# zhong-yy/volpick

Hardware: AMD Instinct MI355X
Metric: waveform-windows/sec (higher is better)
Workload: dtype f32 (exact 3xbf16 split products, fp32 accumulate)

## Files before the change

### include/volpick_hip.h

```cpp
#ifndef VOLPICK_HIP_H
#define VOLPICK_HIP_H

#include <stddef.h>
#include <stdint.h>

#ifdef __cplusplus
extern "C" {
#endif

typedef struct vp_handle vp_handle;

typedef enum {
  VP_OK = 0,
  VP_ERR_INVALID = -1,
  VP_ERR_HIP = -2,
  VP_ERR_NOMEM = -3,
  VP_ERR_UNSUPPORTED = -4
} vp_status;

enum { VP_MODEL_PHASENET = 0, VP_MODEL_EQTRANSFORMER = 1 };
enum { VP_NORM_PEAK = 0, VP_NORM_STD = 1 };
enum { VP_STACK_AVG = 0, VP_STACK_MAX = 1 };
enum { VP_MEM_HOST = 0, VP_MEM_DEVICE = 1 };

// ... 85 lines not shown
int vp_step_issued_work(const vp_handle* h, int index, vp_issued_work* out);
int vp_step_issued_work_for_range(const vp_handle* h, int index, int out_lo, int out_hi, vp_issued_work* out);
int vp_profile_steps(vp_handle* h, int B, int iters, float* step_ms, int cap);
int vp_profile_step_in_pipeline(vp_handle* h, int B, int iters, int index, float* ms);
int vp_profile_one_step(vp_handle* h, int B, int iters, int index, float* ms);

int vp_debug_plan_conv(int model_kind, const float* weights, size_t n_floats, const vp_config* cfg,
                       int conv_index, int* geom13, float* afrag, size_t afrag_cap, float* bias, size_t bias_cap,
                       const char** name, int* cols, int* l_out);

int vp_debug_tensor_count(const vp_handle* h);
int vp_debug_tensor_info(const vp_handle* h, int index, const char** name, int* channels, int* length);
int vp_debug_tensor_read(vp_handle* h, int index, int B, float* host_out);

int vp_debug_check_halos(vp_handle* h, int self_test, int64_t* n_bad, const char** first_bad_tensor);

int vp_debug_core_clock(vp_handle* h, int B, unsigned long long* out32);
int vp_debug_conv_clock(vp_handle* h, unsigned long long* out, int max_layers);
int vp_debug_tail_clock(vp_handle* h, int B, unsigned long long* out32);

enum { VP_SAMPLES_INT32 = 0, VP_SAMPLES_FLOAT32 = 1 };
typedef struct {
  int64_t offset;
  int64_t start_us;
  double sample_rate;
  int32_t reclen, data_offset, nsamples, encoding;
  int32_t big_endian;
  int32_t quality;
  char network[4], station[8], location[4], channel[4];
} vp_mseed_record;
// ... 111 lines not shown
```

### volpick_amd/_lib.py

```python
from __future__ import annotations

import ctypes as C
import os
from pathlib import Path

_HERE = Path(__file__).resolve().parent
LIB_PATH = Path(os.environ.get("VOLPICK_HIP_LIB", _HERE / "libvolpick_hip.so"))

VP_MODEL_PHASENET, VP_MODEL_EQTRANSFORMER = 0, 1
VP_TRAIN_FP32, VP_TRAIN_BF16 = 0, 1
VP_NORM_PEAK, VP_NORM_STD = 0, 1
VP_STACK_AVG, VP_STACK_MAX = 0, 1
VP_MEM_HOST, VP_MEM_DEVICE = 0, 1
VP_MAX_INFLIGHT = 4
VP_ABI_VERSION = 3


class VpConfig(C.Structure):
    _fields_ = [
        ("norm", C.c_int32),
        ("norm_amp_per_comp", C.c_int32),
        ("max_batch", C.c_int32),
        ("bn_eps", C.c_float),
        ("attention_eps", C.c_float),
# ... 216 lines not shown
    "vp_bank_destroy": (C.c_int, [_H]),
    "vp_bank_make_batch": (
        C.c_int, [_H, C.c_void_p, C.c_int, C.c_int, C.c_float, C.c_int, C.POINTER(C.c_int), C.c_void_p, C.c_void_p, C.c_void_p],
    ),
    "vp_train_step_bank": (
        C.c_int,
        [_H, _H, C.c_void_p, C.c_int, C.c_float, C.c_int, C.POINTER(C.c_int), C.c_float, C.c_int, C.POINTER(C.c_double)],
    ),
    "vp_bank_make_batch_aug": (
        C.c_int, [_H, C.c_void_p, C.c_int, C.c_int, C.c_float, C.c_int, C.POINTER(C.c_int), C.c_void_p, C.c_void_p, C.c_void_p],
    ),
    "vp_train_step_bank_aug": (
        C.c_int,
        [_H, _H, C.c_void_p, C.c_int, C.c_float, C.c_int, C.POINTER(C.c_int), C.c_float, C.c_int, C.POINTER(C.c_double)],
    ),
    "vp_last_error": (C.c_char_p, []),
    "vp_version": (C.c_char_p, []),
}


def load():
    global _lib
    if _lib is not None:
        return _lib
    if not LIB_PATH.exists():
        raise VolpickHipError(
            f"{LIB_PATH} not found: the HIP extension is required (no CPU fallback). "
            f"Build it with `make -C {_HERE / 'csrc'}` or `python -c 'import __graft_entry__ as g; g.build()'`."
        )
    try:
# ... 25 lines not shown
```

### volpick_amd/csrc/api.hip

```cpp
#include <algorithm>
#include <cmath>
#include <mutex>
#include <numeric>

#include "net.h"
#include "prepost.h"

namespace vp {
const char* last_error();
}

struct vp_handle {
  int device = 0;
  hipStream_t stream = nullptr;
  vp::Net net;
  hipEvent_t ev[5] = {};
  float total_ms = 0.f;
  bool timing = false;
  float stage_ms[4] = {0.f, 0.f, 0.f, 0.f};
  vp::PreArgs last_pre{};
  int last_pre_windows = 0;
  int last_out_lo = 0, last_out_hi = 0;
  float* d_in = nullptr;
  size_t d_in_cap = 0;
// ... 1076 lines not shown
int vp_debug_tensor_read(vp_handle* h, int index, int B, float* host_out) {
  VP_REQUIRE(h && host_out && index >= 0 && index < (int)h->net.tensors.size(), "bad argument");
  const vp::Tensor& t = h->net.tensors[index];
  if (h->net.tensor_sets[index] == 0) {
    vp::set_error("tensor %s is not materialised by this plan", t.name.c_str());
    return VP_ERR_UNSUPPORTED;
  }
  VP_REQUIRE(B > 0 && B <= h->net.max_batch * h->net.tensor_sets[index], "bad B");
  VP_HIP(hipSetDevice(h->device));
  VP_HIP(hipStreamSynchronize(h->stream));
  VP_HIP(hipMemcpy2D(host_out, (size_t)t.L * sizeof(float), t.p + vp::HALO, (size_t)t.ls * sizeof(float),
                     (size_t)t.L * sizeof(float), (size_t)B * t.C, hipMemcpyDeviceToHost));
  return VP_OK;
}

int vp_debug_check_halos(vp_handle* h, int self_test, int64_t* n_bad, const char** first_bad_tensor) {
  VP_REQUIRE(h && n_bad, "null argument");
  VP_HIP(hipSetDevice(h->device));
  vp::Net& net = h->net;
  const size_t nt = net.tensors.size();
  VP_REQUIRE(self_test >= 0 && self_test <= (int)nt, "self_test names tensor %d of %zu", self_test - 1, nt);
  float* planted = nullptr;
  if (self_test > 0) {
    const vp::Tensor& t = net.tensors[self_test - 1];
    const size_t rows = (size_t)t.C * net.max_batch * net.tensor_sets[self_test - 1];
    VP_REQUIRE(rows > 0, "tensor %s is not materialised by this plan", t.name.c_str());
    planted = t.p + (rows - 1) * t.ls + vp::HALO + t.L;
    const float one = 1.f;
    VP_HIP(hipMemcpyAsync(planted, &one, sizeof(float), hipMemcpyHostToDevice, h->stream));
  }
// ... 85 lines not shown
```

### volpick_amd/csrc/eqt.hip

```cpp
#include "eqt_kernels.h"
#include "net.h"

namespace vp {

namespace {

using EQ_e0 = ConvCfg<3, 0, 8, 2, 12, 2, -5, 0, 1, 4, 8, 1, EPI_POOL2, 1>;
using EQ_e1 = ConvCfg<8, 0, 16, 1, 9, 1, -4, 0, 1, 4, 8, 1, EPI_POOL2, 1>;
using EQ_e2 = ConvCfg<16, 0, 16, 1, 7, 1, -3, 0, 1, 4, 6, 1, EPI_POOL2>;
using EQ_e3 = ConvCfg<16, 0, 32, 1, 7, 1, -3, 0, 2, 2, 6, 1, EPI_POOL2>;
using EQ_e4 = ConvCfg<32, 0, 32, 1, 5, 1, -2, 0, 2, 2, 6, 1, EPI_POOL2, 0, 1>;
using EQ_e5 = ConvCfg<32, 0, 64, 1, 5, 1, -2, 0, 4, 1, 6, 1, EPI_POOL2, 0, 1>;
using EQ_e6 = ConvCfg<64, 0, 64, 1, 3, 1, -1, 0, 4, 1, 3, 1, EPI_POOL2_DUAL, 0, 1>;
using EQ_r1k3 = ConvCfg<64, 0, 64, 1, 3, 1, -1, 0, 4, 1, 3, 1, EPI_STORE>;
using EQ_r1k2 = ConvCfg<64, 0, 64, 1, 2, 1, 0, 0, 4, 1, 3, 1, EPI_STORE>;
using EQ_r2k3 = ConvCfg<64, 0, 64, 1, 3, 1, -1, 0, 4, 1, 3, 0, EPI_RES>;
using EQ_r2k2 = ConvCfg<64, 0, 64, 1, 2, 1, 0, 0, 4, 1, 3, 0, EPI_RES>;
using EQ_d0 = ConvCfg<16, 0, 64, 2, 3, 1, -1, 0, 4, 1, 3, 1, EPI_STORE>;
using EQ_d1 = ConvCfg<64, 0, 64, 2, 3, 1, -1, 0, 4, 1, 6, 1, EPI_STORE, 0, 1>;
using EQ_d2 = ConvCfg<64, 0, 32, 2, 3, 1, -1, 0, 2, 2, 6, 1, EPI_STORE, 0, 1>;
using EQ_d3 = ConvCfg<32, 0, 32, 2, 5, 1, -2, 0, 2, 2, 6, 1, EPI_STORE>;
using EQ_d4 = ConvCfg<32, 0, 16, 2, 5, 1, -2, 0, 2, 2, 6, 1, EPI_STORE, 0, 1>;
using EQ_d5 = ConvCfg<16, 0, 16, 2, 5, 1, -2, 0, 2, 2, 6, 1, EPI_STORE, 0, 1>;
using EQ_d6 = ConvCfg<16, 0, 8, 2, 7, 1, -3, 0, 1, 4, 6, 1, EPI_HEAD, 1>;
// ... 442 lines not shown
    for (int d = 0; d < 3; ++d) {
      const float* hw = pv.get(std::string(head[d]) + ".weight");
      L->e0.h.insert(L->e0.h.end(), hw, hw + 88);
      L->e1.h.push_back(pv.get(std::string(head[d]) + ".bias")[0]);
    }
    L->flops_per_window += 3 * 2.0 * 8 * 11 * T;
    net.steps.back().flops_per_window = L->flops_per_window;
    net.steps.back().name = "decoder.6+heads";
    L->name = "decoder.6";
  }

  net.flops_per_window = 0;
  for (auto& s : net.steps) net.flops_per_window += s.flops_per_window;
  if (net.cfg.plan_flags[1] & 2)
    net.debug_clock = net.add_blob(std::vector<float>(((size_t)net.max_batch * 64 + 64 * 8) * 2, 0.f));
  if (net.cfg.plan_flags[0] != 1) {
    int rc = plan_eqt_fuse_res(net);
    if (rc != VP_OK) return rc;
  }
  if (!(net.cfg.plan_flags[7] & 1) && !alt) {
    int rc = (net.cfg.plan_flags[7] & 64) ? plan_eqt_fuse_tail(net) : plan_eqt_fuse_tail_b3(net);
    if (rc != VP_OK) return rc;
  }
  if (!(net.cfg.plan_flags[7] & 4)) {
    int rc = plan_eqt_fuse_front(net, !(net.cfg.plan_flags[7] & 256));
    if (rc != VP_OK) return rc;
  }
  if (!(net.cfg.plan_flags[7] & 8)) {
    int rc = (net.cfg.plan_flags[7] & 128) ? plan_eqt_fuse_enc36(net) : plan_eqt_fuse_enc36_b3(net);
    if (rc != VP_OK) return rc;
// ... 10 lines not shown
```

### volpick_amd/csrc/eqt_front.hip

```cpp
#include <type_traits>

#include "conv_b3.h"
#include "conv_lds.h"
#include "eqt_kernels.h"
#include "net.h"
#include "prepost.h"

namespace vp {

namespace {

constexpr int FR_NTH = 512, FR_WAVES = 8;
constexpr int FW = 250, FR_TILES = 3;
constexpr int T_IN = 6000, L0P = 3000, L1P = 1500;
using F_e0 = LdsLayer<3, 0, 8, 2, 12, 2, -5, 0, 8, 1>;
using F_e1 = LdsLayer<8, 0, 16, 1, 9, 1, -4, 0, 8, 1>;
using F_e2 = LdsLayer<16, 0, 16, 1, 7, 1, -3, 0, 4, 1>;
constexpr int C0 = 1024, C1 = 1024, C2 = 512;
constexpr int SI = 2065, BII = 8, S0P = 1040, S1P = 528, BI = 4;
static_assert(SI % 32 == 17 && S0P % 32 == 16 && S1P % 32 == 16, "bank-conflict-free strides");
static_assert(SI >= BII + 2 * (C0 - 1) + 12 - 5 && S0P >= BI + C1 + 4 && S0P >= C0 && S1P >= BI + C2 + 3 && S1P >= 1 + C1 / 2,
              "image widths");
constexpr int OFFI = 0, OFF0P = 4 * SI + 4 - (4 * SI) % 4, OFF1P = OFF0P + 8 * S0P, FR_LDS_FLOATS = OFF1P + 16 * S1P;
static_assert(FR_LDS_FLOATS * 4 <= 160 * 1024 && OFF0P % 4 == 0 && OFF1P % 4 == 0, "LDS budget");
// ... 9 lines not shown

struct FrontArgs {
  const float* x;
  int ls_x;
  long ws_x;
  float* y;
  int ls_y;
  long ws_y;
  const float* af[3];
  const float* bs[3];
  const uint4* af3[2];
  int n_tiles;
  PreArgs pre;
  int has_pre;
  int B;
};
struct FrontDumpArgs : FrontArgs {
  float* dbg[2];
  int dbg_ls[2];
  long dbg_ws[2];
};

__device__ __forceinline__ void front_window_stats(const PreArgs& p, const float* src, const long cs, float* red, float* out) {
  constexpr int VT = 1024, NWV = 16, MAXE = 6;
  const int tid = threadIdx.x, lane = tid & 63, wave = tid >> 6, T = p.T;
  float* stat = red + 3 * NWV;
  if (p.norm == VP_NORM_PEAK) {
    float s[2][3], hi[3] = {-INFINITY, -INFINITY, -INFINITY}, lo[3] = {INFINITY, INFINITY, INFINITY};
#pragma unroll
    for (int h = 0; h < 2; ++h)
// ... 222 lines not shown
  float* lds = reinterpret_cast<float*>(fr_lds_raw);
  int off0 = OFF0P / 4, off1 = OFF1P / 4;
  asm volatile("" : "+v"(off0), "+v"(off1));
  float* XI = lds + OFFI;
  float* E0P = lds + 4 * off0;
  float* E1P = lds + 4 * off1;
  bf16_t* E0 = reinterpret_cast<bf16_t*>(reinterpret_cast<char*>(fr_lds_raw) + FB_OFF_E0);
  bf16_t* E1 = reinterpret_cast<bf16_t*>(reinterpret_cast<char*>(fr_lds_raw) + FB_OFF_E1);
  __shared__ float fr_red[3 * 16 + 8 + 3 * 16];
  __shared__ float fr_stat[8];
  const int tid = threadIdx.x, lane = tid & 63;
  const int wave_u = __builtin_amdgcn_readfirstlane(tid >> 6);
  constexpr bool has_pre = CUT;
  int seq = 0;
  auto tile_at = [&](const int q) {
    return has_pre ? ((int)blockIdx.x + (q / FR_TILES) * (int)gridDim.x) * FR_TILES + q % FR_TILES : (int)blockIdx.x + q * (int)gridDim.x;
  };
  int tile = tile_at(0);
  if (tile >= a.n_tiles) return;
  for (int i = tid; i < SI + 4; i += FR_NTH) XI[3 * SI + i] = 0.f;
  if constexpr (B3) {
    uint4* z = reinterpret_cast<uint4*>(reinterpret_cast<char*>(fr_lds_raw) + FB_OFF_E0);
    for (int i = tid; i < (FB_LDS_BYTES - FB_OFF_E0) / 16; i += FR_NTH) z[i] = make_uint4(0u, 0u, 0u, 0u);
  }

  float pre[PRE];
  auto raw_window = [&](const int win, long& cs) -> const float* {
    const PreArgs& p = a.pre;
    long start = p.dense ? 0 : (long)(p.first_window + win) * p.step;
    if (!p.dense && start > p.N - T_IN) start = p.N - T_IN;
    const float* src = p.src + (p.dense ? (long)win * 3 * T_IN : start);
// ... 193 lines not shown
  st.run = [=](Net& n, int B, hipStream_t s) -> int {
    FrontArgs a{};
    const Tensor &tx = n.tensors[x_in], &ty = n.tensors[y_out];
    a.x = tx.p;
    a.ls_x = tx.ls;
    a.ws_x = (long)tx.win_stride();
    a.y = ty.p;
    a.ls_y = ty.ls;
    a.ws_y = (long)ty.win_stride();
    for (int i = 0; i < 3; ++i) {
      a.af[i] = c[i]->afrag.d;
      a.bs[i] = c[i]->bias.d;
    }
    a.n_tiles = B * FR_TILES;
    a.B = B;
    if (n.pre) {
      a.pre = *n.pre;
      a.has_pre = 1;
    }
    const int grid = a.has_pre ? (B < 256 ? B : 256) : (a.n_tiles < 256 ? a.n_tiles : 256);
    if (b3) {
      for (int i = 0; i < 2; ++i) a.af3[i] = reinterpret_cast<const uint4*>(p3[i]->d);
      if (dumps) {
        if (a.has_pre) {
          set_error("fused encoder front: dumps with the in-kernel preprocessing");
          return VP_ERR_UNSUPPORTED;
        }
        FrontDumpArgs d{};
        static_cast<FrontArgs&>(d) = a;
        for (int i = 0; i < 2; ++i) {
// ... 34 lines not shown
```

### volpick_amd/csrc/phasenet_arena.h

```cpp
#pragma once
#include "conv_lds.h"
#include "conv_valu.h"
#include "net.h"

namespace vp {

constexpr int T0 = 3001, T1 = 751, T2 = 188, T3 = 47, T4 = 12;
constexpr int IB = 4;

constexpr int img_stride(int L) { return ((4 + L + 20 - 16 + 31) / 32) * 32 + 16; }
constexpr int S1_ = img_stride(T1), S2_ = img_stride(T2), S3_ = img_stride(T3), S4_ = img_stride(T4);
static_assert(S1_ == 784 && S2_ == 240 && S3_ == 80 && S4_ == 48, "image strides");

template <int C, int S, int L, int B = IB>
__device__ __forceinline__ void zero_halo(float* img, int tid, int nth) {
  constexpr int RW = S - L;
  for (int i = tid; i < C * RW; i += nth) {
    const int c = i / RW, k = i - c * RW;
    img[c * S + (k < B ? k : L + k)] = 0.f;
  }
}

template <int S, int B>
struct RangeStore {
// ... 166 lines not shown
  const uint4* af3_u3t;
  const uint4* af3_u3s;
  const float *bs_u3t, *bs_u3s;
  const float* x;
  int ls_x;
  long ws_x;
  float* skip0;
  int ls_s;
  long ws_s;
  float* y;
  const f32x2 *w_inc, *b_inc, *w_same, *b_same, *w_up, *b_up;
  const float *af_down, *bs_down, *af_t, *bs_t;
  const float *w_out, *b_out;
  PreArgs pre;
  int has_pre;
  float* dbg[WD_COUNT];
  int dbg_ls[WD_COUNT];
  long dbg_ws[WD_COUNT];
};

enum class PnForm {
  Default,
  Level0Valu,
  Fp32Core,
};

void pn_launch_down0(const Down0Args& a, int B, hipStream_t s);
void pn_launch_down0v(const Down0VArgs& a, int B, hipStream_t s);
void pn_launch_core(const CoreArgs& a, int B, hipStream_t s);
void pn_launch_up3(const Up3Args& a, int B, bool persistent, hipStream_t s);
// ... 7 lines not shown
```

### volpick_amd/csrc/phasenet_fused.hip

```cpp
#include "phasenet_arena.h"

namespace vp {

namespace {

int tensor_id(const Net& net, const std::string& name) {
  for (size_t i = 0; i < net.tensors.size(); ++i)
    if (net.tensors[i].name == name) return (int)i;
  return -1;
}

std::vector<float> pack_valu(const float* W, int cin, bool transposed, const std::vector<float>& scale) {
  std::vector<float> out((size_t)cin * 7 * 8);
  for (int ci = 0; ci < cin; ++ci)
    for (int k = 0; k < 7; ++k)
      for (int co = 0; co < 8; ++co)
        out[((size_t)ci * 7 + k) * 8 + co] = scale[co] * (transposed ? W[((size_t)ci * 8 + co) * 7 + k] : W[((size_t)co * cin + ci) * 7 + k]);
  return out;
}

std::vector<float> pack_u2same_half(const ConvLayer& L, int half) {
  const int taps = L.g.taps;
  std::vector<uint16_t> o((size_t)4 * 3 * 64 * 8);
  for (int st = 0; st < 4; ++st)
// ... 217 lines not shown
    a.b_inc = pairs(p.vb[0]);
    a.w_same = pairs(p.vw[1]);
    a.b_same = pairs(p.vb[1]);
    a.w_up = pairs(p.vw[4]);
    a.b_up = pairs(p.vb[4]);
    a.af_down = n.convs[2]->afrag.d;
    a.bs_down = n.convs[2]->bias.d;
    a.af_t = n.convs[16]->afrag.d;
    a.bs_t = n.convs[16]->bias.d;
    a.w_out = e0->d;
    a.b_out = e1->d;
    if (n.pre) {
      a.pre = *n.pre;
      a.has_pre = 1;
    }
    for (size_t i = 0; i < wd_ids.size(); ++i) bind(n.tensors[wd_ids[i]], &a.dbg[i], &a.dbg_ls[i], &a.dbg_ws[i]);
    pn_launch_window(form, !wd_ids.empty(), a, B, s);
    return 0;
  };
  return st;
}

}

int plan_phasenet_fused(Net& net, const ParamView& pv, int debug_flags) {
  PnPlan p{};
  p.debug_dumps = (debug_flags & 1) != 0;
  p.debug_clock = (debug_flags & 2) != 0;
  const bool win_dumps = (debug_flags & 4) != 0;
  const int f5 = net.cfg.plan_flags[5];
  if (win_dumps && (p.debug_dumps || f5 != 0 || net.cfg.plan_flags[6] != 0)) {
    set_error("PhaseNet plan_flags[1] & 4 dumps the default one-launch form only (plan_flags[1] & 1, plan_flags[5], plan_flags[6] unset)");
    return VP_ERR_UNSUPPORTED;
  }
  if (net.cfg.plan_flags[2] == 1 || f5 == 4 || f5 == 5 || f5 == 6 || f5 == 7 || f5 == 9) {
    set_error("PhaseNet plan_flags[2] = %d / plan_flags[5] = %d: this A/B form was removed in round 6 (kept: plan_flags[5] = 0, 1, 2, 3, 8)",
              net.cfg.plan_flags[2], f5);
    return VP_ERR_UNSUPPORTED;
  }
  if (net.cfg.plan_flags[3] == 2) {
    set_error("PhaseNet plan_flags[3] = 2 (persistent level-0 down kernel): removed in round 6");
    return VP_ERR_UNSUPPORTED;
  }
  p.valu = f5 != 1;
  p.persistent = net.cfg.plan_flags[3] != 1;
  const bool whole = p.valu && f5 != 2 && !p.debug_dumps;
  const PnForm form = f5 == 3 ? PnForm::Fp32Core : f5 == 8 ? PnForm::Level0Valu : PnForm::Default;
  if (p.valu) {
    const float eps = net.cfg.bn_eps;
    struct {
      const char *conv, *bn;
      int cin;
      bool transposed, bias;
    } spec[5] = {{"inc", "in_bn", 3, false, true},
                 {"down_branch.0.0", "down_branch.0.1", 8, false, false},
                 {"down_branch.0.2", "down_branch.0.3", 8, false, false},
// ... 60 lines not shown
```

### volpick_amd/csrc/phasenet_window.hip

```cpp
#include "conv_b3.h"
#include "phasenet_arena.h"

namespace vp {

namespace {

constexpr int W0_Q = W0_S / 4;
constexpr int W_LANES = (T0 + 3) / 4;
constexpr int W_WAVES = (W0_Q + 63) / 64;
constexpr int WD_H = 0, WD_X = 8 * W0_S;
static_assert(11 * W0_S <= CORE_LDS_FLOATS, "level-0 down images must fit the core arena");
static_assert(WD_X <= A_D0 && A_D0 + 8 * S1_ <= 11 * W0_S, "down0.down lands on the dead x rows");
constexpr int WU_U = A_SKIP2, WU_G0 = 0, WU_G1 = WU_U + 16 * S1_;
static_assert(WU_G0 + 4 * W0_S <= WU_U && WU_U + 16 * S1_ <= A_U2T && WU_G1 + 4 * W0_S <= CORE_LDS_FLOATS, "up-phase regions");
using W_down = LdsLayer<8, 0, 8, 2, 11, 8, -3, 0, 1, 1>;
using W_upT = LdsLayer<16, 0, 8, 4, 2, 1, -1, -2, 3, 1>;

__device__ __forceinline__ float* win_dump_row(const WindowArgs& a, const int i, const int win, const int c) {
  return a.dbg[i] + (long)win * a.dbg_ws[i] + HALO + (long)c * a.dbg_ls[i];
}
__device__ __forceinline__ float b3_join(const bf16_t* p, const int ps) {
  return from_bf16(p[0]) + (from_bf16(p[ps]) + from_bf16(p[2 * ps]));
}
template <int C, int S, int B>
// ... 47 lines not shown
constexpr int B3_U1_NC = 200, B3_U1_PS = B3_U1_NC * 40;
static_assert(A_U2T * 4 % 16 == 0 && A_U2T * 2 + 3 * B3_U1_PS <= CORE_LDS_FLOATS * 2 && B3_U1_NC >= 192 + 6, "up1.same piece image");
constexpr int B3_U0S_NC = 50, B3_U0S_PS = B3_U0S_NC * 72;
constexpr int B3_U0T_SHIFT = ((A_Q * 2 + 3 * B3_U0S_PS - A_R * 2 + 7) / 8) * 8;
constexpr int B3_U1S_NC = 194;
constexpr int B3_U2_NC = 768, B3_U2_OFF = (A_SKIP2 * 4 + 3 * B3Chunk<32, B3_U1S_NC>::PS * 2 + 15) / 16 * 4;
static_assert(B3_U0T_SHIFT >= 0 && A_R * 2 + B3_U0T_SHIFT + 3 * B3_U0T_PS <= B3_SK3_OFF && (A_R * 2 + B3_U0T_SHIFT) % 8 == 0,
              "up0.convT's image between up0.same's output pieces and the skip-3 image");
static_assert(B3_U2_OFF * 4 + 3 * B3Chunk<16, B3_U2_NC>::PS * 2 <= CORE_LDS_FLOATS * 4 && B3_U2_NC >= 47 * 16 + 8 + 3 &&
                  B3_U1S_NC >= 192 + 2,
              "up1.same's output pieces and up2.same's image behind them fit the arena");
constexpr int B3_D0_NC = 760, B3_D1_NC = 200;
static_assert(A_D0 * 4 + 3 * B3Chunk<8, B3_D0_NC>::PS * 2 <= CORE_LDS_FLOATS * 4 && B3_D0_NC >= 47 * 16 + 7 && B3_D1_NC >= 192 + 7,
              "down0.down / down1.down as piece images");
constexpr int D0T_TS = 512, D0T_RING = 1040, D0T_HPS = B3Chunk<8, D0T_RING>::PS;
constexpr int D0T_RED = CORE_LDS_FLOATS - 256;
static_assert(D0T_TILES * D0T_TS >= W0_S - 4 + 8 && D0T_RING >= 2 * D0T_TS + 11 + 4 && D0T_RING % 2 == 0 &&
                  WD_X * 4 + 3 * D0T_HPS * 2 <= D0T_RED * 4 && (9 * 16 + 8) <= 256,
              "level-0 tiles: the ring behind the eight fp32 rows, the scratch behind the ring, inside the arena");
constexpr int U3T_TS = 256, U3T_RING = 528, U3T_NCU = 768;
using U3T_QU = B3Chunk<16, U3T_NCU>;
constexpr int U3T_PLN = U3T_RING / 2, U3T_MIR = 4;
constexpr int U3T_PL = (U3T_PLN + U3T_MIR) * 8, U3T_CH = 2 * U3T_PL, U3T_PS = 2 * U3T_CH;
constexpr int U3T_RING_OFF = 3 * U3T_QU::PS;
static_assert(U3T_TILES * U3T_TS >= T0 + 8 && U3T_TILES * U3T_TS < 6 * U3T_RING && U3T_RING >= 2 * U3T_TS + 11 + 4 && U3T_NCU >= T1 + 2 &&
                  (U3T_RING_OFF + 3 * U3T_PS) * 2 <= CORE_LDS_FLOATS * 4 && U3T_RING_OFF % 8 == 0,
              "level-0 up tiles: up2.same's piece image and the ring behind it fit the arena");
#define WIN_STAMP(slot) \
  if (clk && tid == 0) clk[(long)win * 32 + (slot)] = __builtin_readcyclecounter();
#ifdef D0T_PROBE
constexpr bool D0T_PROBE_BUILD = true;
#else
constexpr bool D0T_PROBE_BUILD = false;
#endif
#ifdef U3T_PROBE
constexpr bool U3T_PROBE_BUILD = true;
#else
constexpr bool U3T_PROBE_BUILD = false;
#endif
#define CORE_WIN_STAMP(slot) \
  if constexpr (!D0T_PROBE_BUILD && !U3T_PROBE_BUILD) { WIN_STAMP(slot) }
#define D0T_PHASE_STAMP(j) \
  if constexpr (D0T_PROBE_BUILD) { WIN_STAMP(2 + (j)) }
#define U3T_PHASE_STAMP(j) \
  if constexpr (U3T_PROBE_BUILD) { WIN_STAMP(2 + (j)) }

template <PnForm F, bool DUMP = false>
__global__ __launch_bounds__(1024) __attribute__((amdgpu_num_vgpr(60))) void pn_window_kernel(const WindowArgs a) {
  constexpr bool B3 = F != PnForm::Fp32Core;
  constexpr bool D0T = F == PnForm::Default;
  static_assert(!DUMP || F == PnForm::Default, "DUMP instances exist for the default form only");
  constexpr int XU_U = B3 ? A_SKIP1 : WU_U, XU_G0 = B3 ? A_SKIP2 : WU_G0, XU_G1 = B3 ? A_SKIP2 + 4 * W0_S : WU_G1;
  static_assert(XU_G1 + 4 * W0_S <= CORE_LDS_FLOATS && XU_U + 16 * S1_ <= (B3 ? XU_G0 : A_U2T), "up-phase regions");
  extern __shared__ float4 lds_raw[];
  float* lds = reinterpret_cast<float*>(lds_raw);
  const int tid = threadIdx.x, lane = tid & 63, wave = __builtin_amdgcn_readfirstlane(tid >> 6), win = blockIdx.x;
  constexpr int NTH = 1024, NWV = 16;
  unsigned long long* clk = a.c.clk;
  if (clk && tid == 0) clk[(long)win * 32 + 16] = wall_clock64();
#define WIN_DUMP(...)   \
  if constexpr (DUMP) { \
    __VA_ARGS__;        \
    __syncthreads();    \
  }
  WIN_STAMP(0)
  WIN_STAMP(18)
  if (win < 8 && a.c.warm) {
    float sink = 0.f;
#define CORE_WARM(IDX, LAYER)                                                                          \
  for (int l = tid; l < LAYER::MT * LAYER::CB * LAYER::TAPS * 2; l += NTH) sink += a.c.af[IDX][l * 32];
    CORE_WARM(0, C_d1same) CORE_WARM(1, C_d1down) CORE_WARM(2, C_d2same) CORE_WARM(3, C_d2down)
    if constexpr (B3) {
#pragma unroll
      for (int i = 0; i < 6; ++i)
        for (int l = tid; l < a.af3_lines[i]; l += NTH) sink += __uint_as_float(reinterpret_cast<const unsigned*>(a.af3[i])[l * 32]);
    } else {
      CORE_WARM(4, C_d3same) CORE_WARM(5, C_d3down) CORE_WARM(6, C_d4same) CORE_WARM(7, C_u0T) CORE_WARM(8, C_u0same)
    }
    CORE_WARM(9, C_u1T) CORE_WARM(10, C_u1same) CORE_WARM(11, C_u2T) CORE_WARM(12, C_u2same)
#undef CORE_WARM
    if (sink == 1.2345678e-30f) a.y[0] = sink;
  }
// ... 14 lines not shown
    float *H = lds + WD_H, *X = lds + WD_X;
    constexpr int MAXE = (T0 + NTH - 1) / NTH;
    float v[3][MAXE];
    [[maybe_unused]] uint4 aI[3], aS[B3Steps<8, 8>::STEPS * 3];
    [[maybe_unused]] f32x4 bI, bS;
    if constexpr (D0T) {
#pragma unroll
      for (int pc = 0; pc < 3; ++pc) aI[pc] = a.af3_inc[pc * 64 + lane];
      b3_load_a<8, 8>(a.af3_d0s, 0, lane, aS);
#pragma unroll
      for (int r = 0; r < 4; ++r) bI[r] = a.bs_inc8[4 * ((lane >> 4) & 1) + r], bS[r] = a.bs_d0s[4 * ((lane >> 4) & 1) + r];
    }
    if (a.has_pre) {
      const PreArgs& p = a.pre;
      float* red = lds + (D0T ? D0T_RED : 11 * W0_S);
      float* stat = red + 9 * NWV;
      long start = p.dense ? 0 : (long)(p.first_window + win) * p.step;
      if (!p.dense && start > p.N - T0) start = p.N - T0;
      const float* src = p.src + (p.dense ? (long)win * 3 * T0 : start);
      long cs = p.dense ? T0 : p.N;
      if (p.table) {
        const long* e = p.table + 3 * (p.first_window + win);
        src = p.src + e[0] + e[2];
        cs = e[1];
      }
      float sum[3] = {0.f, 0.f, 0.f};
#pragma unroll
      for (int c = 0; c < 3; ++c)
#pragma unroll
        for (int k = 0; k < MAXE; ++k) {
          const int t = tid + k * NTH;
          v[c][k] = t < T0 ? src[c * cs + t] : 0.f;
          sum[c] += v[c][k];
        }
      const bool one_pass = p.norm == VP_NORM_PEAK;
      float vhi[3] = {-INFINITY, -INFINITY, -INFINITY}, vlo[3] = {INFINITY, INFINITY, INFINITY};
      if (one_pass) {
#pragma unroll
        for (int c = 0; c < 3; ++c)
#pragma unroll
          for (int k = 0; k < MAXE; ++k)
            if (tid + k * NTH < T0) vhi[c] = fmaxf(vhi[c], v[c][k]), vlo[c] = fminf(vlo[c], v[c][k]);
      }
      wave_sum3(sum[0], sum[1], sum[2]);
      if (one_pass) {
        float nlo[3] = {-vlo[0], -vlo[1], -vlo[2]};
        wave_max3(vhi[0], vhi[1], vhi[2]);
        wave_max3(nlo[0], nlo[1], nlo[2]);
        if (lane == 0)
          for (int c = 0; c < 3; ++c) red[(3 + c) * NWV + wave] = vhi[c], red[(6 + c) * NWV + wave] = -nlo[c];
      }
      if (lane == 0)
        for (int c = 0; c < 3; ++c) red[c * NWV + wave] = sum[c];
      WIN_STAMP(29)
      if constexpr (!D0T) {
        for (int i = tid; i < 3 * (W0_S - T0); i += NTH) {
          const int c = i / (W0_S - T0), k = i - c * (W0_S - T0);
          X[c * W0_S + (k < 4 ? k : T0 + k)] = 0.f;
        }
      }
      __syncthreads();
      if (tid < 3) {
        float acc = 0.f;
        for (int i = 0; i < NWV; ++i) acc += red[tid * NWV + i];
        const float mu = acc / (float)T0;
        stat[tid * 2] = mu;
        if (one_pass) {
          float h = red[(3 + tid) * NWV], l = red[(6 + tid) * NWV];
          for (int i = 1; i < NWV; ++i) h = fmaxf(h, red[(3 + tid) * NWV + i]), l = fminf(l, red[(6 + tid) * NWV + i]);
          stat[tid * 2 + 1] = fmaxf(h - mu, mu - l);
        }
      }
      __syncthreads();
      WIN_STAMP(30)
      const float mean[3] = {stat[0], stat[2], stat[4]};
      if (!one_pass) {
      float m[3] = {0.f, 0.f, 0.f};
#pragma unroll
      for (int c = 0; c < 3; ++c)
#pragma unroll
        for (int k = 0; k < MAXE; ++k) {
          const int t = tid + k * NTH;
          if (t < T0) {
            const float d = v[c][k] - mean[c];
            m[c] = fmaf(d, d, m[c]);
          }
        }
      __syncthreads();
      for (int c = 0; c < 3; ++c) {
        const float r = wave_sum(m[c]);
        if (lane == 0) red[c * NWV + wave] = r;
      }
      __syncthreads();
      if (tid < 3) {
        const float* r = red + tid * NWV;
        float acc = r[0];
        for (int i = 1; i < NWV; ++i) acc = acc + r[i];
        stat[tid * 2 + 1] = acc;
      }
      __syncthreads();
      }
      for (int c = 0; c < 3; ++c) poisoned |= !isfinite(stat[2 * c]) || !isfinite(stat[2 * c + 1]);
      float amp[3];
      if (p.per_comp) {
        for (int c = 0; c < 3; ++c) amp[c] = (p.norm == VP_NORM_PEAK) ? stat[2 * c + 1] : sqrtf(stat[2 * c + 1] / (float)(T0 - 1));
      } else {
        const float g = (p.norm == VP_NORM_PEAK) ? fmaxf(stat[1], fmaxf(stat[3], stat[5]))
                                                 : sqrtf((stat[1] + stat[3] + stat[5]) / (float)(3 * T0 - 1));
        amp[0] = amp[1] = amp[2] = g;
      }
      const NormDiv den[3] = {norm_div_prepare(amp[0] + p.norm_eps), norm_div_prepare(amp[1] + p.norm_eps),
                              norm_div_prepare(amp[2] + p.norm_eps)};
      if (p.taper > 0) {
#pragma unroll
        for (int c = 0; c < 3; ++c)
#pragma unroll
          for (int k = 0; k < MAXE; ++k) {
            const int t = tid + k * NTH;
            if (t < T0) {
              float o = norm_div(v[c][k] - mean[c], den[c]);
              const int e = (t < p.taper) ? t : ((T0 - 1 - t < p.taper) ? T0 - 1 - t : -1);
              if (e >= 0) o *= 0.5f * (1.f + cosf(3.14159265358979323846f * (1.f + (float)e / (float)(p.taper - 1))));
              if constexpr (D0T) v[c][k] = o;
              else X[c * W0_S + 4 + t] = o;
            }
          }
      } else {
#pragma unroll
        for (int c = 0; c < 3; ++c)
#pragma unroll
          for (int k = 0; k < MAXE; ++k) {
            const int t = tid + k * NTH;
            if constexpr (D0T) v[c][k] = norm_div(v[c][k] - mean[c], den[c]);
            else if (k + 1 < MAXE || t < T0) X[c * W0_S + 4 + t] = norm_div(v[c][k] - mean[c], den[c]);
          }
      }
    } else if constexpr (D0T) {
      const float* src = a.x + (long)win * a.ws_x + HALO;
#pragma unroll
      for (int c = 0; c < 3; ++c)
#pragma unroll
        for (int k = 0; k < MAXE; ++k) {
          const int t = tid + k * NTH;
          v[c][k] = t < T0 ? src[(long)c * a.ls_x + t] : 0.f;
        }
    } else {
      const float* src = a.x + (long)win * a.ws_x;
      for (int i = tid; i < 3 * W0_Q; i += NTH) {
        const int c = i / W0_Q, q = i - c * W0_Q;
        const int p = 4 * q + HALO - 4;
        float4 v = make_float4(0.f, 0.f, 0.f, 0.f);
        if (p + 3 < a.ls_x) v = *reinterpret_cast<const float4*>(src + (long)c * a.ls_x + p);
        *reinterpret_cast<float4*>(X + c * W0_S + 4 * q) = v;
      }
    }
    if constexpr (!D0T) {
      if (tid < 8) *reinterpret_cast<float4*>(H + tid * W0_S) = make_float4(0.f, 0.f, 0.f, 0.f);
    } else if (tid < 8) {
      H[tid * W0_S] = H[tid * W0_S + 1] = H[tid * W0_S + 2] = 0.f;
      if (tid >= 6) H[tid * W0_S + 3] = 0.f;
    }
    if constexpr (D0T) {
      bf16_t* const l16 = reinterpret_cast<bf16_t*>(lds);
      bf16_t* const HP = l16 + WD_X * 2;
      unsigned* const HU = reinterpret_cast<unsigned*>(H);
      const int g = lane >> 4, n = lane & 15, ph = g >> 1, quad = g & 1;
#pragma unroll
      for (int k = 0; k < MAXE; ++k) {
        const int t = tid + k * NTH;
        if (k + 1 < MAXE || t < T0) {
          const float q0 = v[0][k], q1 = v[1][k], q2 = v[2][k];
          const unsigned h0 = pack_bf16x2(q0, q1), h1 = pack_bf16x2(q2, 0.f);
          const float r0 = q0 - bf16_lo(h0), r1 = q1 - bf16_hi(h0), r2 = q2 - bf16_lo(h1);
          const unsigned m0 = pack_bf16x2(r0, r1), m1 = pack_bf16x2(r2, 0.f);
          unsigned* const xp = HU + 3 + t;
          xp[0] = h0;
          xp[W0_S] = h1;
          xp[2 * W0_S] = m0;
          xp[3 * W0_S] = m1;
          xp[4 * W0_S] = pack_bf16x2(r0 - bf16_lo(m0), r1 - bf16_hi(m0));
          xp[5 * W0_S] = pack_bf16x2(r2 - bf16_lo(m1), 0.f);
        }
      }
      if (tid < 6 * (W0_S - 3 - T0)) {
        const int r = tid / (W0_S - 3 - T0), c = tid - r * (W0_S - 3 - T0);
        HU[r * W0_S + 3 + T0 + c] = 0u;
      }
      auto ring_at = [](const int c) { return (c & 1) * (D0T_RING / 2 * 8) + (c >> 1) * 8; };
      if (tid < 48)
        *reinterpret_cast<uint4*>(HP + (tid >> 4) * D0T_HPS + ring_at(D0T_RING - 16 + (tid & 15))) = make_uint4(0u, 0u, 0u, 0u);
      const int skip_ch = tid >> 7, skip_q = tid & 127;
      float* const skip_row = a.skip0 + (long)win * a.ws_s + HALO + (long)skip_ch * a.ls_s;
      auto store_skip_tile = [&](const int k) {
        const int ts = D0T_TS * k - 8 + 4 * skip_q;
        if (ts >= 0 && ts < T0)
          *reinterpret_cast<f32x4*>(skip_row + ts) = *reinterpret_cast<const f32x4*>(H + skip_ch * W0_S + 4 + ts);
// ... 743 lines not shown
      float* y = a.y + (long)win * 3 * T0 + t0;
      if (t0 + 3 < T0) {
        *reinterpret_cast<f32x4u*>(y) = y0;
        *reinterpret_cast<f32x4u*>(y + T0) = y1;
        *reinterpret_cast<f32x4u*>(y + 2 * T0) = y2;
      } else {
#pragma unroll
        for (int r = 0; r < 4; ++r)
          if (t0 + r < T0) y[r] = y0[r], y[T0 + r] = y1[r], y[2 * T0 + r] = y2[r];
      }
    }
    WIN_STAMP(28)
  }
  if (clk && tid == 0) clk[(long)win * 32 + 17] = wall_clock64();
#undef WIN_STAMP
#undef CORE_WIN_STAMP
#undef D0T_PHASE_STAMP
#undef U3T_PHASE_STAMP
#undef WIN_DUMP
#undef WIN_WARM_SCALAR
}

}

void pn_launch_window(PnForm form, bool dump, const WindowArgs& a, int B, hipStream_t s) {
  const dim3 grid(B), block(1024);
  const size_t lds = CORE_LDS_FLOATS * sizeof(float);
  if (dump) hipLaunchKernelGGL((pn_window_kernel<PnForm::Default, true>), grid, block, lds, s, a);
  else if (form == PnForm::Default) hipLaunchKernelGGL(pn_window_kernel<PnForm::Default>, grid, block, lds, s, a);
  else if (form == PnForm::Level0Valu) hipLaunchKernelGGL(pn_window_kernel<PnForm::Level0Valu>, grid, block, lds, s, a);
// ... 12 lines not shown
```

### volpick_amd/csrc/vp_common.h

```cpp
#pragma once
#include <hip/hip_runtime.h>

#include <cstdarg>
#include <cstdint>
#include <cstdio>
#include <cstring>
#include <map>
#include <string>
#include <vector>

#include "../../include/volpick_hip.h"

namespace vp {

constexpr int HALO = 8;

typedef float f32x4 __attribute__((ext_vector_type(4)));

void set_error(const char* fmt, ...);

#define VP_HIP(call)                                                                         \
  do {                                                                                       \
    hipError_t e_ = (call);                                                                  \
    if (e_ != hipSuccess) {                                                                  \
      vp::set_error("%s failed: %s (%s:%d)", #call, hipGetErrorString(e_), __FILE__, __LINE__); \
      return VP_ERR_HIP;                                                                     \
    }                                                                                        \
  } while (0)

#define VP_REQUIRE(cond, ...)     \
  do {                            \
    if (!(cond)) {                \
// ... 34 lines not shown
```

Baseline: 3.525 million.

## Place consecutive windows on the same XCD and remove normalisation-stat LDS round trip

Remaps workgroup index to window index so that contiguous windows land on the same XCD (MI355X dispatches workgroups round-robin across 8 XCDs), in both the PhaseNet window kernel and the EQTransformer front kernel. Overlapping input windows then share L2 on one XCD instead of being spread across all of them. The per-window mean and amplitude reduction now has every lane read the partial sums as 16-byte vector loads and broadcasts them with readlane, removing a stat buffer and two __syncthreads. Also adds debug poison and readback APIs and an optional timing-probe build, and new plan flags select the old placement.

```diff
diff --git a/include/volpick_hip.h b/include/volpick_hip.h
--- a/include/volpick_hip.h
+++ b/include/volpick_hip.h
@@ -123,6 +123,9 @@
 int vp_debug_tensor_read(vp_handle* h, int index, int B, float* host_out);
 
 int vp_debug_check_halos(vp_handle* h, int self_test, int64_t* n_bad, const char** first_bad_tensor);
+
+int vp_debug_poison_outputs(vp_handle* h, int tensor);
+int vp_debug_window_predictions(vp_handle* h, int64_t n, float* host_out);
 
 int vp_debug_core_clock(vp_handle* h, int B, unsigned long long* out32);
 int vp_debug_conv_clock(vp_handle* h, unsigned long long* out, int max_layers);
diff --git a/volpick_amd/_lib.py b/volpick_amd/_lib.py
--- a/volpick_amd/_lib.py
+++ b/volpick_amd/_lib.py
@@ -254,6 +254,8 @@
         C.c_int,
         [_H, _H, C.c_void_p, C.c_int, C.c_float, C.c_int, C.POINTER(C.c_int), C.c_float, C.c_int, C.POINTER(C.c_double)],
     ),
+    "vp_debug_poison_outputs": (C.c_int, [_H, C.c_int]),
+    "vp_debug_window_predictions": (C.c_int, [_H, C.c_int64, C.c_void_p]),
     "vp_last_error": (C.c_char_p, []),
     "vp_version": (C.c_char_p, []),
 }
diff --git a/volpick_amd/csrc/api.hip b/volpick_amd/csrc/api.hip
--- a/volpick_amd/csrc/api.hip
+++ b/volpick_amd/csrc/api.hip
@@ -1114,6 +1114,33 @@
   return VP_OK;
 }
 
+int vp_debug_poison_outputs(vp_handle* h, int tensor) {
+  VP_REQUIRE(h && tensor >= -1 && tensor < (int)h->net.tensors.size(), "bad argument");
+  VP_HIP(hipSetDevice(h->device));
+  VP_HIP(hipStreamSynchronize(h->stream));
+  vp::Net& net = h->net;
+  VP_HIP(hipMemset(net.y, 0xFF, (size_t)net.max_batch * net.n_out * net.in_samples * sizeof(float)));
+  if (h->d_pred) VP_HIP(hipMemset(h->d_pred, 0xFF, h->d_pred_cap * sizeof(float)));
+  if (tensor >= 0) {
+    const vp::Tensor& t = net.tensors[tensor];
+    const size_t rows = (size_t)t.C * net.max_batch * net.tensor_sets[tensor];
+    VP_REQUIRE(rows > 0 && t.p, "tensor %s is not materialised by this plan", t.name.c_str());
+    VP_HIP(hipMemset2D(t.p + vp::HALO, (size_t)t.ls * sizeof(float), 0xFF, (size_t)t.L * sizeof(float), rows));
+  }
+  VP_HIP(hipDeviceSynchronize());
+  return VP_OK;
+}
+
+int vp_debug_window_predictions(vp_handle* h, int64_t n, float* host_out) {
+  VP_REQUIRE(h && host_out && n > 0, "bad argument");
+  const size_t need = (size_t)n * h->net.n_out * h->net.in_samples;
+  VP_REQUIRE(h->d_pred && need <= h->d_pred_cap, "no window predictions of %lld windows (run vp_annotate / vp_classify first)", (long long)n);
+  VP_HIP(hipSetDevice(h->device));
+  VP_HIP(hipStreamSynchronize(h->stream));
+  VP_HIP(hipMemcpy(host_out, h->d_pred, need * sizeof(float), hipMemcpyDeviceToHost));
+  return VP_OK;
+}
+
 int vp_debug_check_halos(vp_handle* h, int self_test, int64_t* n_bad, const char** first_bad_tensor) {
   VP_REQUIRE(h && n_bad, "null argument");
   VP_HIP(hipSetDevice(h->device));
diff --git a/volpick_amd/csrc/eqt.hip b/volpick_amd/csrc/eqt.hip
--- a/volpick_amd/csrc/eqt.hip
+++ b/volpick_amd/csrc/eqt.hip
@@ -480,6 +480,11 @@
   for (auto& s : net.steps) net.flops_per_window += s.flops_per_window;
   if (net.cfg.plan_flags[1] & 2)
     net.debug_clock = net.add_blob(std::vector<float>(((size_t)net.max_batch * 64 + 64 * 8) * 2, 0.f));
+  if (net.cfg.plan_flags[5] != 0 && net.cfg.plan_flags[5] != 1) {
+    set_error("EQTransformer plan_flags[5] = %d: unknown window placement (0 = XCD-contiguous, 1 = workgroup b takes window b)",
+              net.cfg.plan_flags[5]);
+    return VP_ERR_UNSUPPORTED;
+  }
   if (net.cfg.plan_flags[0] != 1) {
     int rc = plan_eqt_fuse_res(net);
     if (rc != VP_OK) return rc;
diff --git a/volpick_amd/csrc/eqt_front.hip b/volpick_amd/csrc/eqt_front.hip
--- a/volpick_amd/csrc/eqt_front.hip
+++ b/volpick_amd/csrc/eqt_front.hip
@@ -47,6 +47,7 @@
   PreArgs pre;
   int has_pre;
   int B;
+  int xcd_place;
 };
 struct FrontDumpArgs : FrontArgs {
   float* dbg[2];
@@ -299,7 +300,11 @@
   constexpr bool has_pre = CUT;
   int seq = 0;
   auto tile_at = [&](const int q) {
-    return has_pre ? ((int)blockIdx.x + (q / FR_TILES) * (int)gridDim.x) * FR_TILES + q % FR_TILES : (int)blockIdx.x + q * (int)gridDim.x;
+    if constexpr (!has_pre) return (int)blockIdx.x + q * (int)gridDim.x;
+    const int pass0 = (q / FR_TILES) * (int)gridDim.x, left = a.B - pass0;
+    const int nb = left < (int)gridDim.x ? left : (int)gridDim.x;
+    const int w = (a.xcd_place && (int)blockIdx.x < nb) ? xcd_window((int)blockIdx.x, nb) : (int)blockIdx.x;
+    return (pass0 + w) * FR_TILES + q % FR_TILES;
   };
   int tile = tile_at(0);
   if (tile >= a.n_tiles) return;
@@ -523,6 +528,7 @@
     }
     a.n_tiles = B * FR_TILES;
     a.B = B;
+    a.xcd_place = n.cfg.plan_flags[5] != 1;
     if (n.pre) {
       a.pre = *n.pre;
       a.has_pre = 1;
diff --git a/volpick_amd/csrc/phasenet_arena.h b/volpick_amd/csrc/phasenet_arena.h
--- a/volpick_amd/csrc/phasenet_arena.h
+++ b/volpick_amd/csrc/phasenet_arena.h
@@ -204,6 +204,7 @@
   const float *w_out, *b_out;
   PreArgs pre;
   int has_pre;
+  int xcd_place;
   float* dbg[WD_COUNT];
   int dbg_ls[WD_COUNT];
   long dbg_ws[WD_COUNT];
diff --git a/volpick_amd/csrc/phasenet_fused.hip b/volpick_amd/csrc/phasenet_fused.hip
--- a/volpick_amd/csrc/phasenet_fused.hip
+++ b/volpick_amd/csrc/phasenet_fused.hip
@@ -255,6 +255,7 @@
       a.pre = *n.pre;
       a.has_pre = 1;
     }
+    a.xcd_place = n.cfg.plan_flags[7] != 1;
     for (size_t i = 0; i < wd_ids.size(); ++i) bind(n.tensors[wd_ids[i]], &a.dbg[i], &a.dbg_ls[i], &a.dbg_ws[i]);
     pn_launch_window(form, !wd_ids.empty(), a, B, s);
     return 0;
@@ -281,6 +282,10 @@
   }
   if (net.cfg.plan_flags[3] == 2) {
     set_error("PhaseNet plan_flags[3] = 2 (persistent level-0 down kernel): removed in round 6");
+    return VP_ERR_UNSUPPORTED;
+  }
+  if (net.cfg.plan_flags[7] != 0 && net.cfg.plan_flags[7] != 1) {
+    set_error("PhaseNet plan_flags[7] = %d: unknown window placement (0 = XCD-contiguous, 1 = workgroup b takes window b)", net.cfg.plan_flags[7]);
     return VP_ERR_UNSUPPORTED;
   }
   p.valu = f5 != 1;
diff --git a/volpick_amd/csrc/phasenet_window.hip b/volpick_amd/csrc/phasenet_window.hip
--- a/volpick_amd/csrc/phasenet_window.hip
+++ b/volpick_amd/csrc/phasenet_window.hip
@@ -85,6 +85,7 @@
 static_assert(A_D0 * 4 + 3 * B3Chunk<8, B3_D0_NC>::PS * 2 <= CORE_LDS_FLOATS * 4 && B3_D0_NC >= 47 * 16 + 7 && B3_D1_NC >= 192 + 7,
               "down0.down / down1.down as piece images");
 constexpr int D0T_TS = 512, D0T_RING = 1040, D0T_HPS = B3Chunk<8, D0T_RING>::PS;
+static_assert(CORE_LDS_FLOATS % 4 == 0 && (11 * W0_S) % 4 == 0, "the reduction scratch is read in 16-byte words");
 constexpr int D0T_RED = CORE_LDS_FLOATS - 256;
 static_assert(D0T_TILES * D0T_TS >= W0_S - 4 + 8 && D0T_RING >= 2 * D0T_TS + 11 + 4 && D0T_RING % 2 == 0 &&
                   WD_X * 4 + 3 * D0T_HPS * 2 <= D0T_RED * 4 && (9 * 16 + 8) <= 256,
@@ -109,8 +110,18 @@
 #else
 constexpr bool U3T_PROBE_BUILD = false;
 #endif
+#ifdef LOADX_PROBE
+constexpr bool LOADX_PROBE_BUILD = true;
+#else
+constexpr bool LOADX_PROBE_BUILD = false;
+#endif
 #define CORE_WIN_STAMP(slot) \
   if constexpr (!D0T_PROBE_BUILD && !U3T_PROBE_BUILD) { WIN_STAMP(slot) }
+#define LOADX_STAMP(slot, PRE)           \
+  if constexpr (LOADX_PROBE_BUILD) {     \
+    if (clk) { PRE; }                    \
+    WIN_STAMP(slot)                      \
+  }
 #define D0T_PHASE_STAMP(j) \
   if constexpr (D0T_PROBE_BUILD) { WIN_STAMP(2 + (j)) }
 #define U3T_PHASE_STAMP(j) \
@@ -125,7 +136,8 @@
   static_assert(XU_G1 + 4 * W0_S <= CORE_LDS_FLOATS && XU_U + 16 * S1_ <= (B3 ? XU_G0 : A_U2T), "up-phase regions");
   extern __shared__ float4 lds_raw[];
   float* lds = reinterpret_cast<float*>(lds_raw);
-  const int tid = threadIdx.x, lane = tid & 63, wave = __builtin_amdgcn_readfirstlane(tid >> 6), win = blockIdx.x;
+  const int tid = threadIdx.x, lane = tid & 63, wave = __builtin_amdgcn_readfirstlane(tid >> 6);
+  const int win = a.xcd_place ? xcd_window((int)blockIdx.x, (int)gridDim.x) : (int)blockIdx.x;
   constexpr int NTH = 1024, NWV = 16;
   unsigned long long* clk = a.c.clk;
   if (clk && tid == 0) clk[(long)win * 32 + 16] = wall_clock64();
@@ -136,7 +148,7 @@
   }
   WIN_STAMP(0)
   WIN_STAMP(18)
-  if (win < 8 && a.c.warm) {
+  if (blockIdx.x < XCDS && a.c.warm) {
     float sink = 0.f;
 #define CORE_WARM(IDX, LAYER)                                                                          \
   for (int l = tid; l < LAYER::MT * LAYER::CB * LAYER::TAPS * 2; l += NTH) sink += a.c.af[IDX][l * 32];
@@ -181,7 +193,6 @@
     if (a.has_pre) {
       const PreArgs& p = a.pre;
       float* red = lds + (D0T ? D0T_RED : 11 * W0_S);
-      float* stat = red + 9 * NWV;
       long start = p.dense ? 0 : (long)(p.first_window + win) * p.step;
       if (!p.dense && start > p.N - T0) start = p.N - T0;
       const float* src = p.src + (p.dense ? (long)win * 3 * T0 : start);
@@ -200,6 +211,7 @@
           v[c][k] = t < T0 ? src[c * cs + t] : 0.f;
           sum[c] += v[c][k];
         }
+      LOADX_STAMP(15, asm volatile("s_waitcnt vmcnt(0)" ::: "memory"))
       const bool one_pass = p.norm == VP_NORM_PEAK;
       float vhi[3] = {-INFINITY, -INFINITY, -INFINITY}, vlo[3] = {INFINITY, INFINITY, INFINITY};
       if (one_pass) {
@@ -227,20 +239,28 @@
         }
       }
       __syncthreads();
-      if (tid < 3) {
+      auto from_lane = [](const float x, const int l) { return __int_as_float(__builtin_amdgcn_readlane(__float_as_int(x), l)); };
+      float mean[3], second[3];
+      {
+        const f32x4* rp = reinterpret_cast<const f32x4*>(red + (lane < 9 ? lane : 8) * NWV);
+        f32x4 q[NWV / 4];
+#pragma unroll
+        for (int i = 0; i < NWV / 4; ++i) q[i] = rp[i];
         float acc = 0.f;
-        for (int i = 0; i < NWV; ++i) acc += red[tid * NWV + i];
+#pragma unroll
+        for (int i = 0; i < NWV; ++i) acc += q[i / 4][i % 4];
         const float mu = acc / (float)T0;
-        stat[tid * 2] = mu;
+#pragma unroll
+        for (int c = 0; c < 3; ++c) mean[c] = from_lane(mu, c);
         if (one_pass) {
-          float h = red[(3 + tid) * NWV], l = red[(6 + tid) * NWV];
-          for (int i = 1; i < NWV; ++i) h = fmaxf(h, red[(3 + tid) * NWV + i]), l = fminf(l, red[(6 + tid) * NWV + i]);
-          stat[tid * 2 + 1] = fmaxf(h - mu, mu - l);
-        }
-      }
-      __syncthreads();
+          float h = q[0][0], l = q[0][0];
+#pragma unroll
+          for (int i = 1; i < NWV; ++i) h = fmaxf(h, q[i / 4][i % 4]), l = fminf(l, q[i / 4][i % 4]);
+#pragma unroll
+          for (int c = 0; c < 3; ++c) second[c] = fmaxf(from_lane(h, 3 + c) - mean[c], mean[c] - from_lane(l, 6 + c));
+        }
+      }
       WIN_STAMP(30)
-      const float mean[3] = {stat[0], stat[2], stat[4]};
       if (!one_pass) {
       float m[3] = {0.f, 0.f, 0.f};
 #pragma unroll
@@ -259,21 +279,26 @@
         if (lane == 0) red[c * NWV + wave] = r;
       }
       __syncthreads();
-      if (tid < 3) {
-        const float* r = red + tid * NWV;
-        float acc = r[0];
-        for (int i = 1; i < NWV; ++i) acc = acc + r[i];
-        stat[tid * 2 + 1] = acc;
-      }
-      __syncthreads();
-      }
-      for (int c = 0; c < 3; ++c) poisoned |= !isfinite(stat[2 * c]) || !isfinite(stat[2 * c + 1]);
+      {
+        const f32x4* rp = reinterpret_cast<const f32x4*>(red + (lane < 3 ? lane : 2) * NWV);
+        float acc = 0.f;
+#pragma unroll
+        for (int i = 0; i < NWV / 4; ++i) {
+          const f32x4 q = rp[i];
+#pragma unroll
+          for (int r = 0; r < 4; ++r) acc = (i == 0 && r == 0) ? q[r] : acc + q[r];
+        }
+#pragma unroll
+        for (int c = 0; c < 3; ++c) second[c] = from_lane(acc, c);
+      }
+      }
+      for (int c = 0; c < 3; ++c) poisoned |= !isfinite(mean[c]) || !isfinite(second[c]);
       float amp[3];
       if (p.per_comp) {
-        for (int c = 0; c < 3; ++c) amp[c] = (p.norm == VP_NORM_PEAK) ? stat[2 * c + 1] : sqrtf(stat[2 * c + 1] / (float)(T0 - 1));
+        for (int c = 0; c < 3; ++c) amp[c] = (p.norm == VP_NORM_PEAK) ? second[c] : sqrtf(second[c] / (float)(T0 - 1));
       } else {
-        const float g = (p.norm == VP_NORM_PEAK) ? fmaxf(stat[1], fmaxf(stat[3], stat[5]))
-                                                 : sqrtf((stat[1] + stat[3] + stat[5]) / (float)(3 * T0 - 1));
+        const float g = (p.norm == VP_NORM_PEAK) ? fmaxf(second[0], fmaxf(second[1], second[2]))
+                                                 : sqrtf((second[0] + second[1] + second[2]) / (float)(3 * T0 - 1));
         amp[0] = amp[1] = amp[2] = g;
       }
       const NormDiv den[3] = {norm_div_prepare(amp[0] + p.norm_eps), norm_div_prepare(amp[1] + p.norm_eps),
@@ -302,6 +327,7 @@
             else if (k + 1 < MAXE || t < T0) X[c * W0_S + 4 + t] = norm_div(v[c][k] - mean[c], den[c]);
           }
       }
+      LOADX_STAMP(26, asm volatile("" ::"v"(v[0][0]), "v"(v[1][1]), "v"(v[2][MAXE - 1])))
     } else if constexpr (D0T) {
       const float* src = a.x + (long)win * a.ws_x + HALO;
 #pragma unroll
@@ -332,21 +358,43 @@
       bf16_t* const HP = l16 + WD_X * 2;
       unsigned* const HU = reinterpret_cast<unsigned*>(H);
       const int g = lane >> 4, n = lane & 15, ph = g >> 1, quad = g & 1;
-#pragma unroll
-      for (int k = 0; k < MAXE; ++k) {
-        const int t = tid + k * NTH;
-        if (k + 1 < MAXE || t < T0) {
+      if constexpr (!LOADX_PROBE_BUILD) {
+#pragma unroll
+        for (int k = 0; k < MAXE; ++k) {
+          const int t = tid + k * NTH;
+          if (k + 1 < MAXE || t < T0) {
+            const float q0 = v[0][k], q1 = v[1][k], q2 = v[2][k];
+            const unsigned h0 = pack_bf16x2(q0, q1), h1 = pack_bf16x2(q2, 0.f);
+            const float r0 = q0 - bf16_lo(h0), r1 = q1 - bf16_hi(h0), r2 = q2 - bf16_lo(h1);
+            const unsigned m0 = pack_bf16x2(r0, r1), m1 = pack_bf16x2(r2, 0.f);
+            unsigned* const xp = HU + 3 + t;
+            xp[0] = h0;
+            xp[W0_S] = h1;
+            xp[2 * W0_S] = m0;
+            xp[3 * W0_S] = m1;
+            xp[4 * W0_S] = pack_bf16x2(r0 - bf16_lo(m0), r1 - bf16_hi(m0));
+            xp[5 * W0_S] = pack_bf16x2(r2 - bf16_lo(m1), 0.f);
+          }
+        }
+      } else {
+        unsigned pw[MAXE][6];
+#pragma unroll
+        for (int k = 0; k < MAXE; ++k) {
           const float q0 = v[0][k], q1 = v[1][k], q2 = v[2][k];
           const unsigned h0 = pack_bf16x2(q0, q1), h1 = pack_bf16x2(q2, 0.f);
           const float r0 = q0 - bf16_lo(h0), r1 = q1 - bf16_hi(h0), r2 = q2 - bf16_lo(h1);
           const unsigned m0 = pack_bf16x2(r0, r1), m1 = pack_bf16x2(r2, 0.f);
-          unsigned* const xp = HU + 3 + t;
-          xp[0] = h0;
-          xp[W0_S] = h1;
-          xp[2 * W0_S] = m0;
-          xp[3 * W0_S] = m1;
-          xp[4 * W0_S] = pack_bf16x2(r0 - bf16_lo(m0), r1 - bf16_hi(m0));
-          xp[5 * W0_S] = pack_bf16x2(r2 - bf16_lo(m1), 0.f);
+          pw[k][0] = h0, pw[k][1] = h1, pw[k][2] = m0, pw[k][3] = m1;
+          pw[k][4] = pack_bf16x2(r0 - bf16_lo(m0), r1 - bf16_hi(m0));
+          pw[k][5] = pack_bf16x2(r2 - bf16_lo(m1), 0.f);
+        }
+        LOADX_STAMP(27, asm volatile("" ::"v"(pw[0][4]), "v"(pw[1][5]), "v"(pw[MAXE - 1][4])))
+#pragma unroll
+        for (int k = 0; k < MAXE; ++k) {
+          const int t = tid + k * NTH;
+          if (k + 1 < MAXE || t < T0)
+#pragma unroll
+            for (int r = 0; r < 6; ++r) HU[3 + t + r * W0_S] = pw[k][r];
         }
       }
       if (tid < 6 * (W0_S - 3 - T0)) {
@@ -1120,6 +1168,7 @@
   }
   if (clk && tid == 0) clk[(long)win * 32 + 17] = wall_clock64();
 #undef WIN_STAMP
+#undef LOADX_STAMP
 #undef CORE_WIN_STAMP
 #undef D0T_PHASE_STAMP
 #undef U3T_PHASE_STAMP
diff --git a/volpick_amd/csrc/vp_common.h b/volpick_amd/csrc/vp_common.h
--- a/volpick_amd/csrc/vp_common.h
+++ b/volpick_amd/csrc/vp_common.h
@@ -16,6 +16,15 @@
 constexpr int HALO = 8;
 
 typedef float f32x4 __attribute__((ext_vector_type(4)));
+
+constexpr int XCDS = 8;
+__host__ __device__ constexpr int xcd_window(const int b, const int nb) {
+  const int q = nb / XCDS, r = nb % XCDS, x = b % XCDS;
+  return x * q + (x < r ? x : r) + b / XCDS;
+}
+static_assert(xcd_window(0, 9) == 0 && xcd_window(8, 9) == 1 && xcd_window(1, 9) == 2 && xcd_window(7, 9) == 8 && xcd_window(255, 256) == 255 &&
+                  xcd_window(1, 256) == 32 && xcd_window(4, 5) == 4,
+              "xcd_window");
 
 void set_error(const char* fmt, ...);
 
```

After: 3.513 million. Within noise of the previous version (-0.3%).
